# zju3dv/BoxDreamer

Hardware: AMD Instinct MI355X
Metric: poses/s/GPU (5-ref, 224×224, bf16); heatmap max-abs err vs CPU ref (higher is better)
Workload: dtype f16 + e4m3 corrections (BETR q, k columns: f16)

## Files before the change

### boxdreamer_amd/_lib.py

```python
from __future__ import annotations

import ctypes as C
import os
import threading
from typing import NamedTuple

import torch

HERE = os.path.dirname(os.path.abspath(__file__))
LIB_PATH = os.environ.get("BOXDREAMER_HIP_LIB") or os.path.join(HERE, "libboxdreamer_hip.so")

DTYPE_BF16, DTYPE_F16, DTYPE_F32 = 0, 1, 2
PREC_BF16, PREC_F16, PREC_BF16X3, PREC_F16_OUT_BF16X3, PREC_FP8, PREC_BF16_OUT_FP8 = 0, 1, 2, 3, 4, 5
PREC_BF16X3_ATTN_X3 = 6
PREC_F16C8 = 8
PREC_F16_OUT_F16C8, PREC_BF16X3_OUT_F16C8 = 9, 10
PREC_F16C8_QK16 = 13
PREC_F16X3, PREC_F16X3_ATTN_X3 = 14, 15
PREC_F16_OUT_F16X3, PREC_BF16X3_OUT_F16X3 = 16, 17
F16C8_D = 11
PREC_NAMES = {"bf16": PREC_BF16, "fp16": PREC_F16, "f16": PREC_F16, "bf16x3": PREC_BF16X3, "fp8": PREC_FP8,
              "bf16x3_attn_x3": PREC_BF16X3_ATTN_X3, "f16c8": PREC_F16C8, "f16c8_qk16": PREC_F16C8_QK16,
              "f16x3": PREC_F16X3, "f16x3_attn_x3": PREC_F16X3_ATTN_X3}
PREC_NAMES["fp8_mixed"] = PREC_FP8
# ... 60 lines not shown


class BetrWeights(C.Structure):
    _fields_ = [("depth", C.c_int), ("dim", C.c_int), ("heads", C.c_int), ("grid", C.c_int),
                ("patch", C.c_int), ("box_dim", C.c_int), ("kpad", C.c_int),
                ("ln_eps", C.c_float), ("adapter_ln_eps", C.c_float), ("rms_eps", C.c_float),
                ("adapter_fc1", Linear), ("adapter_fc2", Linear), ("bbox_emb", Linear), ("bbox_proj", Linear),
                ("pos_table", C.c_void_p), ("query_token", C.c_void_p),
                ("blocks", C.POINTER(BlockWeights)), ("promote_misc", C.c_int), ("latency_mode", C.c_int)]


class TraceRecord(C.Structure):
    _fields_ = [("kind", C.c_int), ("M", C.c_int), ("N", C.c_int), ("K", C.c_int), ("ms", C.c_float)]


EXPORTS = [
    "bd_abi_version", "bd_target_arch", "bd_gemm", "bd_layernorm", "bd_qk_rmsnorm", "bd_attention",
    "bd_im2col_images", "bd_patchify_heatmaps", "bd_write_prefix_tokens", "bd_query_substitute",
    "bd_gather_query_tokens", "bd_unpatchify_sigmoid", "bd_decode_topk",
    "bd_encoder_workspace_bytes", "bd_encoder_forward", "bd_decoder_workspace_bytes", "bd_decoder_forward",
    "bd_trace_begin", "bd_trace_end", "bd_render_corner_heatmaps", "bd_attention_q", "bd_gather_query_rows_f32",
    "bd_dino_match_scores", "bd_topk_mask", "bd_solve_pnp", "bd_gemm_fuses_qk_rmsnorm", "bd_gemm_takes_ln_fold", "bd_gemm_splitk_flag_bytes",
    "bd_gemm_splitk_workspace_bytes", "bd_solve_pnp_host", "bd_attention_prefix",
    "bd_lanes_prepare", "bd_encoder_workspace_bytes_lanes", "bd_encoder_forward_lanes", "bd_decoder_workspace_bytes_lanes",
    "bd_decoder_forward_lanes", "bd_pose_metrics_workspace_bytes", "bd_pose_metrics", "bd_crop_resize_frames",
    "bd_attention_varlen", "bd_query_substitute_varlen", "bd_gather_query_rows_f32_varlen", "bd_gather_query_tokens_varlen",
    "bd_decoder_workspace_bytes_ragged", "bd_decoder_forward_ragged", "bd_gather_view_rows",
    "bd_match_view_sums", "bd_match_select_rows",
    "bd_assemble_entry_tokens", "bd_decoder_entry_tokens_workspace_bytes", "bd_decoder_entry_tokens",
    "bd_decoder_entry_workspace_bytes", "bd_decoder_forward_entry", "bd_decoder_entry_workspace_bytes_ragged",
    "bd_decoder_forward_entry_ragged", "bd_solve_pnp_wave",
    "bd_solve_pnp_ransac_workspace_bytes", "bd_solve_pnp_ransac_wave", "bd_solve_pnp_ransac_host",
    "bd_round_sources", "bd_pose_select_rows",
]

_lib = None


def load() -> C.CDLL:
    global _lib
    _call.dev = None
    if _lib is not None:
        return _lib
    if not os.path.exists(LIB_PATH):
        raise HipLibraryError(
            f"{LIB_PATH} is missing: the gfx950 HIP kernels are not built. Run "
            "`python -m boxdreamer_amd.build` (or __graft_entry__.build()). There is no CPU/PyTorch fallback.")
    lib = C.CDLL(LIB_PATH)
    for name in EXPORTS:
        if not hasattr(lib, name):
            raise HipLibraryError(f"{LIB_PATH} does not export {name}")
    i, i64, vp, f, sz = C.c_int, C.c_int64, C.c_void_p, C.c_float, C.c_size_t
    lib.bd_abi_version.restype = i
    lib.bd_target_arch.restype = C.c_char_p
    lib.bd_gemm.argtypes = [C.POINTER(GemmArgs), i, vp]
    lib.bd_gemm_fuses_qk_rmsnorm.argtypes = [C.POINTER(GemmArgs), i]
    lib.bd_gemm_takes_ln_fold.argtypes = [C.POINTER(GemmArgs), i]
    lib.bd_gemm_splitk_flag_bytes.argtypes = [i, i]
    lib.bd_gemm_splitk_flag_bytes.restype = sz
    lib.bd_gemm_splitk_workspace_bytes.argtypes = [i, i]
    lib.bd_gemm_splitk_workspace_bytes.restype = sz
    lib.bd_layernorm.argtypes = [vp, i64, vp, vp, f, vp, i64, vp, i64, i, i, i, i, i, i, vp]
    lib.bd_qk_rmsnorm.argtypes = [vp, i64, vp, vp, f, i, i, i, i, vp]
    lib.bd_attention.argtypes = [vp, i64, vp, i64, i, i, i, i, f, i, vp]
    lib.bd_im2col_images.argtypes = [vp, i, vp, i64, i, i, i, i, i, vp]
    lib.bd_patchify_heatmaps.argtypes = [vp, i, vp, i64, i, i, i, i, i, i, vp]
    lib.bd_write_prefix_tokens.argtypes = [vp, vp, i, i, i, i, vp]
    lib.bd_query_substitute.argtypes = [vp, vp, vp, vp, vp, i, i, i, i, vp]
    lib.bd_gather_query_tokens.argtypes = [vp, vp, vp, i64, i, i, i, i, i, vp]
    lib.bd_unpatchify_sigmoid.argtypes = [vp, vp, vp, i, i, i, i, vp]
    lib.bd_decode_topk.argtypes = [vp, i, i, i, i, vp, vp, vp, vp]
    lib.bd_encoder_workspace_bytes.argtypes = [C.POINTER(DinoWeights), i, i]
    lib.bd_encoder_workspace_bytes.restype = sz
    lib.bd_encoder_forward.argtypes = [C.POINTER(DinoWeights), vp, i, i, i, vp, vp, i64, vp, sz, i, vp]
    lib.bd_decoder_workspace_bytes.argtypes = [C.POINTER(BetrWeights), i, i, i]
    lib.bd_decoder_workspace_bytes.restype = sz
    lib.bd_decoder_forward.argtypes = [C.POINTER(BetrWeights), vp, i, vp, i64, vp, i, i, i, vp, vp, vp, sz, i, vp]
    lib.bd_encoder_workspace_bytes_lanes.argtypes = [C.POINTER(DinoWeights), i, i, i]
    lib.bd_encoder_workspace_bytes_lanes.restype = sz
    lib.bd_encoder_forward_lanes.argtypes = [C.POINTER(DinoWeights), vp, i, i, i, vp, vp, i64, vp, sz, i, i, vp]
    lib.bd_decoder_workspace_bytes_lanes.argtypes = [C.POINTER(BetrWeights), i, i, i, i]
    lib.bd_decoder_workspace_bytes_lanes.restype = sz
    lib.bd_decoder_forward_lanes.argtypes = [C.POINTER(BetrWeights), vp, i, vp, i64, vp, i, i, i, vp, vp, vp, sz, i, i, vp]
    lib.bd_lanes_prepare.argtypes = []
    lib.bd_attention_q.argtypes = [vp, i64, vp, i64, i, i, i, i, f, vp, i, i, vp]
    lib.bd_attention_prefix.argtypes = [vp, i64, vp, i64, i, i, i, i, f, i, i, i, vp]
    lib.bd_gather_query_rows_f32.argtypes = [vp, vp, vp, i, i, i, i, vp]
    lib.bd_render_corner_heatmaps.argtypes = [vp, i, i, i, i, vp, i, vp]
    lib.bd_dino_match_scores.argtypes = [vp, vp, i, vp, i, i, i, i, i, i, f, vp, vp, vp, vp]
    lib.bd_topk_mask.argtypes = [vp, i, i, i, vp, vp]
# ... 291 lines not shown
```

### boxdreamer_amd/csrc/bd_common.h

```cpp
#pragma once
#include <hip/hip_runtime.h>
#include <stdint.h>

#include "../../include/boxdreamer_hip.h"

typedef __attribute__((__vector_size__(8 * sizeof(__bf16)))) __bf16 bf16x8;
typedef __attribute__((__vector_size__(8 * sizeof(_Float16)))) _Float16 f16x8;
typedef __attribute__((__vector_size__(16 * sizeof(float)))) float f32x16;
typedef __attribute__((__vector_size__(4 * sizeof(float)))) float f32x4;
typedef __attribute__((__vector_size__(16))) unsigned int u128;

template <class T> struct Op16;
template <> struct Op16<__bf16> {
    typedef bf16x8 vec8;
    static __device__ __forceinline__ f32x16 mfma(vec8 a, vec8 b, f32x16 c) {
        return __builtin_amdgcn_mfma_f32_32x32x16_bf16(a, b, c, 0, 0, 0);
    }
};
template <> struct Op16<_Float16> {
    typedef f16x8 vec8;
    static __device__ __forceinline__ f32x16 mfma(vec8 a, vec8 b, f32x16 c) {
        return __builtin_amdgcn_mfma_f32_32x32x16_f16(a, b, c, 0, 0, 0);
    }
};
// ... 286 lines not shown
            }
            if (beta) {
                const float4 bb = *(const float4*)(beta + c);
                y[0] += bb.x; y[1] += bb.y; y[2] += bb.z; y[3] += bb.w;
            }
            if (out32_row) *(float4*)(out32_row + c) = make_float4(y[0], y[1], y[2], y[3]);
            if (out16) {
                if constexpr (__is_same(T, f16c8)) {
                    f16c8_store4(out16, out16_plane, orow * cols + c, y);
                } else if constexpr (NS == 2) {
                    float hi4[4], lo4[4];
#pragma unroll
                    for (int j = 0; j < 4; ++j) split_hi_lo<T>(y[j], hi4[j], lo4[j]);
                    store_cvt<T, 4>(out16 + orow * cols + c, hi4);
                    store_cvt<T, 4>(out16 + out16_plane + orow * cols + c, lo4);
                } else {
                    store_cvt<T, 4>(out16 + orow * cols + c, y);
                }
            }
        }
    }
}

template <class T, int NS, bool NT>
__device__ __forceinline__ void ln_row(const float* __restrict__ xr, const float* __restrict__ gamma, const float* __restrict__ beta,
                                       float eps, T* __restrict__ out16, int64_t out16_plane, float* __restrict__ out32_row,
                                       int64_t orow, int cols, int lane) {
    f32x4 t[4];
    ln_row_load<NT>(xr, cols, lane, t);
    ln_row_finish<T, NS>(t, gamma, beta, eps, out16, out16_plane, out32_row, orow, cols, lane);
}

int& bd_concurrent_launches();

int bd_attention_q_forms(const void* qkv, int64_t qkv_plane, void* out, int64_t out_plane, int batch, int seq, int heads, int head_dim,
                         float scale, const int32_t* q_view, int q_len, int prec, int latency_forms, void* stream);

int bd_assemble_entry_tokens_from(const float* bank_x, int bank_views, const float* rgb_fresh, int fresh_first, int n_fresh, const float* pos,
                                  const float* query_token, const int32_t* src, float* x_out, int n_views, int P, int dim, void* stream);

int bd_trace_open(hipStream_t s, int kind, int M, int N, int K);
void bd_trace_close(hipStream_t s, int slot);

#define BD_CHECK_LAUNCH() do { hipError_t e__ = hipGetLastError(); if (e__ != hipSuccess) return (int)e__; } while (0)
```

### boxdreamer_amd/csrc/gemm_common.h

```cpp
#pragma once
#include "bd_common.h"
#include <type_traits>

#ifdef BD_GEMM_PROBE
static __device__ unsigned* bd_probe_buf = nullptr;
#define BD_PROBE(idx) { const unsigned long long t__ = __builtin_amdgcn_s_memtime(); if ((idx) < 64) probe_ts = (lane == (idx)) ? (unsigned)t__ : probe_ts; }
#define BD_PROBE_IF(c, idx) { if (c) BD_PROBE(idx) }
#define BD_PROBE_RT(idx) { const unsigned long long t__ = __builtin_amdgcn_s_memrealtime(); probe_ts = (lane == (idx)) ? (unsigned)t__ : probe_ts; }
#else
#define BD_PROBE(idx)
#define BD_PROBE_IF(c, idx)
#define BD_PROBE_RT(idx)
#endif


namespace {


template <int CH> __device__ __forceinline__ int swz_chunk(int row, int c) {
    constexpr int RPB = 16 / CH;
    return c ^ ((row / RPB) & (CH - 1));
}

template <int BM_, int BN_>
// ... 654 lines not shown
    const float m[8] = {st[0][0], st[0][2], st[1][0], st[1][2], st[2][0], st[2][2], st[3][0], st[3][2]};
    const float q[8] = {st[0][1], st[0][3], st[1][1], st[1][3], st[2][1], st[2][3], st[3][1], st[3][3]};
    float mean = 0.f, m2 = 0.f;
#pragma unroll
    for (int i = 0; i < 8; ++i) mean += m[i];
    mean *= 0.125f;
#pragma unroll
    for (int i = 0; i < 8; ++i) { const float d = m[i] - mean; m2 += q[i] + 96.0f * (d * d); }
    const float rstd = rsqrtf(m2 * (1.0f / 768.0f) + eps);
    return make_float2(rstd, -mean * rstd);
}
inline bool ln_fold_producer(const bd_gemm_args& a) { return a.ln_stats_out != nullptr || a.ln_op_out != nullptr || a.ln_resid_in_op != 0; }
inline bool ln_fold_consumer(const bd_gemm_args& a) { return a.ln_stats_in != nullptr || a.ln_colsum != nullptr; }
inline bool ln_fold_producer_ok(const bd_gemm_args& a) {
    if (a.ln_resid_in_op ? (a.resid != nullptr || (a.out_f32 != OUT_F32 && a.out_f32 != OUT_OPERAND)) : a.out_f32 != OUT_F32) return false;
    return a.ln_stats_out && a.ln_op_out && a.N == 768 && a.act == BD_ACT_NONE && !a.rms_wq && !a.addtab && a.rpg_in <= 0 &&
           !a.wscale && a.ln_op_ld % 32 == 0 && a.ln_op_plane % 8 == 0 && (((uintptr_t)a.ln_op_out | (uintptr_t)a.ln_stats_out) & 15) == 0 &&
           (int64_t)a.M * a.ln_op_ld < ((int64_t)1 << 30);
}
inline bool ln_fold_consumer_ok(const bd_gemm_args& a) {
    return a.ln_stats_in && a.ln_colsum && a.K == 768 && a.N % 192 == 0 && a.out_f32 != OUT_F32 && !a.resid && !a.addtab && a.rpg_in <= 0 && !a.wscale &&
           a.bias && (((uintptr_t)a.ln_stats_in | (uintptr_t)a.ln_colsum | (uintptr_t)a.bias) & 15) == 0;
}

inline bool wide_epilogue_ok(const bd_gemm_args& p, int ns) {
    return (p.N % 8 == 0) && (p.ldo % 8 == 0) && (((uintptr_t)p.out & 15) == 0) &&
           (!p.resid || ((p.ldr % 4 == 0) && ((uintptr_t)p.resid & 15) == 0)) &&
           (!p.bias || ((uintptr_t)p.bias & 15) == 0) && (!p.addtab || ((uintptr_t)p.addtab & 15) == 0) &&
           (!p.wscale || ((uintptr_t)p.wscale & 15) == 0) && (p.out_f32 || ns == 1 || (p.out_plane % 8 == 0));
}


inline int cu_count() {
    static int cached[16] = {0};
    int dev = 0;
    if (hipGetDevice(&dev) != hipSuccess || dev < 0 || dev >= 16) return 256;
    if (cached[dev] == 0) {
        int n = 0;
        if (hipDeviceGetAttribute(&n, hipDeviceAttributeMultiprocessorCount, dev) != hipSuccess || n <= 0) n = 256;
        cached[dev] = n;
    }
    return cached[dev];
}

inline bool rms_geometry_ok(const bd_gemm_args& a) {
    return a.rms_wq && a.rms_wk && a.out_f32 != OUT_F32 && a.act == BD_ACT_NONE && !a.resid && !a.addtab && a.rpg_in <= 0 &&
           (a.rms_parts == 0 || a.rms_parts == 2 || a.rms_parts == 3) &&
           a.N % (a.rms_parts == 2 ? 2 : 3) == 0 && (a.N / (a.rms_parts == 2 ? 2 : 3)) % 96 == 0 && a.N % 192 == 0 && (((uintptr_t)a.rms_wq | (uintptr_t)a.rms_wk) & 3) == 0;
}

}

inline int64_t pc192_main_rows(const bd_gemm_args& a, int cus) {
    if (a.rms_wq || a.addtab || a.rpg_in > 0) return a.M;
    const int64_t tn = a.N / 192, mt = (a.M + 255) / 256, nt = mt * tn;
    const int64_t k = nt / cus, rem = nt % cus;
    if (k < 1 || k > 4 || rem == 0 || rem * 4 > cus) return a.M;
    const int64_t rows = (k * cus / tn) * 256;
    return rows > 0 ? rows : a.M;
}

int bd_launch_gemm_f16c8(const bd_gemm_args& a, hipStream_t s);
bool bd_f16c8_takes_ln_fold(const bd_gemm_args& a);
```

### boxdreamer_amd/csrc/gemm_f16c8.hip

```cpp
#include "gemm_common.h"

#ifdef BD_GEMM_PROBE
extern "C" int bd_gemm_f16c8_probe_set(void* buf) {
    return (int)hipMemcpyToSymbol(HIP_SYMBOL(bd_probe_buf), &buf, sizeof(buf));
}
#endif

namespace {

template <int NSTAGE, int EP, int OUTK, bool GELU, int WM = 4, int WN = 2, int NPW = 4, bool LNF = false, bool SK = false>
__global__ __launch_bounds__((WM * WN + NPW) * 64, (WM * WN + NPW) <= 4 ? 2 : 1) void gemm_kernel_pc_f16c8(const bd_gemm_args p) {
    constexpr int MI = 2, NI = 3, NCW = WM * WN;
    constexpr int TBM = WM * MI * 32, TBN = WN * NI * 32, BK = 32;
    constexpr int A0 = TBM * 64, W0 = TBN * 64, A1 = TBM * 32, W1 = TBN * 64;
    constexpr int OFF_W0 = A0, OFF_A1 = A0 + W0, OFF_W1 = A0 + W0 + A1, STAGE = A0 + W0 + A1 + W1;
    constexpr int SR = 16, SCRATCH = NCW * SR * NI * 32 * 4, S2 = SCRATCH > STAGE ? SCRATCH : STAGE;
    static_assert(SCRATCH <= STAGE, "the epilogue scratch overlays stage 2");
    constexpr int GA0 = TBM / 16, GW0 = TBN / 16, GA1 = TBM / 32, GW1 = TBN / 16;
    constexpr int IA0 = (GA0 + NPW - 1) / NPW, IW0 = (GW0 + NPW - 1) / NPW, IA1 = (GA1 + NPW - 1) / NPW, IW1 = (GW1 + NPW - 1) / NPW;
    static_assert(GA0 % NPW == 0 && GW0 % NPW == 0 && GA1 % NPW == 0 && GW1 % NPW == 0, "every producer wave issues the same number of pieces (counted vmcnt)");
    constexpr int PIECES = IA0 + IW0 + IA1 + IW1;
    constexpr int WAIT_ONE_SLAB = (PIECES & 15) | ((PIECES >> 4) << 14) | 0x70 | 0xF00;
    constexpr int AUX_COLP = 2 * STAGE + S2, AUX_RMS = AUX_COLP + 4096, AUX_ROWS = AUX_RMS + 2048, AUX_BYTES = EP == 0 ? 0 : (LNF ? 10240 : 6144);
    static_assert(!LNF || (EP != 0 && NPW * 64 >= TBM && NSTAGE == 3), "LayerNorm fold: one producer lane per tile row");
// ... 344 lines not shown
                          (ep == 2 && outk == OUT_F16);
        if (!form) return false;
    }
    return true;
}

static int f16c8_split_k(const bd_gemm_args& a, int ep, bool r5, bool lnp, bool s3, int cus) {
    (void)lnp;
    if (!a.sk_ws || ((uintptr_t)a.sk_ws & 255) || !s3 || a.N % 96 != 0 || !bd_gemm_splitk_flag_bytes(a.M, a.N) || !(ep == 3 || r5)) return 1;
    const int t96 = ((a.M + 127) / 128) * (a.N / 96), nk = a.K / 32;
    const int slots = cus / (bd_concurrent_launches() > 0 ? bd_concurrent_launches() : 1);
    int sk = a.sk_split;
    if (sk <= 0) {
        sk = 1;
        for (int c = 4; c >= 2; --c)
            if (t96 * c <= slots && nk / c >= 6) { sk = c; break; }
    }
    if (sk < 2 || sk > 4 || nk / sk < 1) return 1;
    return sk;
}

extern "C" size_t bd_gemm_splitk_flag_bytes(int M, int N) {
    if (M <= 0 || N <= 0 || N % 96 != 0 || M > BD_SPLITK_MAX_ROWS) return 0;
    const size_t t96 = (size_t)((M + 127) / 128) * (size_t)(N / 96);
    return t96 * 3 * 2 * 4 <= BD_SPLITK_FLAG_BYTES ? BD_SPLITK_FLAG_BYTES : 0;
}
extern "C" size_t bd_gemm_splitk_workspace_bytes(int M, int N) {
    const size_t fb = bd_gemm_splitk_flag_bytes(M, N);
    if (!fb) return 0;
    const size_t t96 = (size_t)((M + 127) / 128) * (size_t)(N / 96);
    return fb + t96 * 3 * 2 * (size_t)(64 * 96 * 4);
}

int bd_launch_gemm_f16c8(const bd_gemm_args& a, hipStream_t s) {
    if (!wide_epilogue_ok(a, 2) || 256 * a.lda * 2 >= ((int64_t)1 << 31) || 256 * a.ldw * 2 >= ((int64_t)1 << 31)) return BD_ERR_ALIGN;
    if ((a.K % 32) || (a.lda % 32) || (a.ldw % 32)) return BD_ERR_SHAPE;
    if (a.out_f32 == OUT_OPERAND && (a.ldo % 32)) return BD_ERR_SHAPE;
    if (a.w_qexp + BD_F16C8_D < -100 || a.w_qexp + BD_F16C8_D > 120) return BD_ERR_SHAPE;
    if (a.rms_wq && !rms_geometry_ok(a)) return BD_ERR_SHAPE;
    const bool lnp = ln_fold_producer(a), lnc = ln_fold_consumer(a);
    if ((lnp || lnc) && !bd_f16c8_takes_ln_fold(a)) return BD_ERR_SHAPE;
    const int slot = bd_trace_open(s, 0, a.M, a.N, a.K);
    const int cus = cu_count();
    const int tiles = ((a.M + 255) / 256) * ((a.N + 191) / 192);
    int outk = 0;
    bool gelu = false;
    const int ep = f16c8_epilogue_kind(a, outk, gelu);
    const bool s3 = (a.K / 32) % 3 == 0;
    const int tiles_small = ((a.M + 127) / 128) * ((a.N + 191) / 192);
    const bool small = s3 && ep != 0 && 2 * tiles * bd_concurrent_launches() <= cus;
    const bool small0 = ep == 0 && 2 * tiles * bd_concurrent_launches() <= cus;
    const dim3 g0(tiles_small < cus ? tiles_small : cus);
    const int grid = small ? (tiles_small < cus ? tiles_small : cus) : (tiles < cus ? tiles : cus);
    const dim3 g(grid), b(small ? 512 : 768);
#define BD_C8_LAUNCH(EP_, OUTK_, GELU_)                                                                     \
    { if (small) hipLaunchKernelGGL((gemm_kernel_pc_f16c8<3, EP_, OUTK_, GELU_, 2, 2, 4>), g, b, 0, s, a);     \
      else if (s3) hipLaunchKernelGGL((gemm_kernel_pc_f16c8<3, EP_, OUTK_, GELU_>), g, b, 0, s, a);            \
      else hipLaunchKernelGGL((gemm_kernel_pc_f16c8<2, EP_, OUTK_, GELU_>), g, b, 0, s, a); }
#define BD_C8_LAUNCH_LN(EP_, OUTK_, GELU_, LNF_)                                                                        \
    { if (small) hipLaunchKernelGGL((gemm_kernel_pc_f16c8<3, EP_, OUTK_, GELU_, 2, 2, 4, LNF_>), g, b, 0, s, a);         \
      else hipLaunchKernelGGL((gemm_kernel_pc_f16c8<3, EP_, OUTK_, GELU_, 4, 2, 4, LNF_>), g, b, 0, s, a); }
    const bool r5 = lnp && a.ln_resid_in_op;
    const bool fc2_96 = (ep == 3 || r5) && small && a.K >= 2048 && a.N % 96 == 0 && 4 * tiles * bd_concurrent_launches() <= cus;
    const int sk = f16c8_split_k(a, ep, r5, lnp, s3, cus);
    if (sk > 1) {
        bd_gemm_args b2 = a;
        b2.sk_split = sk;
        const int t96 = ((a.M + 127) / 128) * (a.N / 96);
        const dim3 gs(((t96 + 7) / 8) * 8 * sk), bs(256);
        if (r5 && a.out_f32 == OUT_F32) hipLaunchKernelGGL((gemm_kernel_pc_f16c8<3, 5, OUT_F32, false, 2, 1, 2, false, true>), gs, bs, 0, s, b2);
        else if (r5) hipLaunchKernelGGL((gemm_kernel_pc_f16c8<3, 5, OUT_OPERAND, false, 2, 1, 2, false, true>), gs, bs, 0, s, b2);
        else if (lnp) hipLaunchKernelGGL((gemm_kernel_pc_f16c8<3, 4, OUT_F32, false, 2, 1, 2, false, true>), gs, bs, 0, s, b2);
        else hipLaunchKernelGGL((gemm_kernel_pc_f16c8<3, 3, OUT_F32, false, 2, 1, 2, false, true>), gs, bs, 0, s, b2);
        bd_trace_close(s, slot);
        BD_CHECK_LAUNCH();
        return BD_OK;
    }
    if (r5 && fc2_96 && a.out_f32 == OUT_F32)
        hipLaunchKernelGGL((gemm_kernel_pc_f16c8<3, 5, OUT_F32, false, 2, 1, 2>), dim3(((a.M + 127) / 128) * (a.N / 96)), dim3(256), 0, s, a);
    else if (r5 && fc2_96)
        hipLaunchKernelGGL((gemm_kernel_pc_f16c8<3, 5, OUT_OPERAND, false, 2, 1, 2>), dim3(((a.M + 127) / 128) * (a.N / 96)), dim3(256), 0, s, a);
    else if (r5 && a.out_f32 == OUT_F32) BD_C8_LAUNCH_LN(5, OUT_F32, false, false)
    else if (r5) BD_C8_LAUNCH_LN(5, OUT_OPERAND, false, false)
    else if (lnp && fc2_96)
        hipLaunchKernelGGL((gemm_kernel_pc_f16c8<3, 4, OUT_F32, false, 2, 1, 2>), dim3(((a.M + 127) / 128) * (a.N / 96)), dim3(256), 0, s, a);
    else if (lnp) BD_C8_LAUNCH_LN(4, OUT_F32, false, false)
    else if (lnc && ep == 1 && gelu) BD_C8_LAUNCH_LN(1, OUT_OPERAND, true, true)
    else if (lnc && ep == 1 && outk == OUT_F16) BD_C8_LAUNCH_LN(1, OUT_F16, false, true)
    else if (lnc && ep == 1) BD_C8_LAUNCH_LN(1, OUT_BF16X2, false, true)
    else if (lnc) BD_C8_LAUNCH_LN(2, OUT_F16, false, true)
    else if (fc2_96)
        hipLaunchKernelGGL((gemm_kernel_pc_f16c8<3, 3, OUT_F32, false, 2, 1, 2>), dim3(((a.M + 127) / 128) * (a.N / 96)), dim3(256), 0, s, a);
    else if (ep == 3) BD_C8_LAUNCH(3, OUT_F32, false)
    else if (ep == 2 && outk == OUT_OPERAND) BD_C8_LAUNCH(2, OUT_OPERAND, false)
    else if (ep == 2 && outk == OUT_F16) BD_C8_LAUNCH(2, OUT_F16, false)
    else if (ep == 2) BD_C8_LAUNCH(2, OUT_BF16X2, false)
    else if (ep == 1 && gelu) BD_C8_LAUNCH(1, OUT_OPERAND, true)
    else if (ep == 1 && outk == OUT_OPERAND) BD_C8_LAUNCH(1, OUT_OPERAND, false)
    else if (ep == 1 && outk == OUT_F16) BD_C8_LAUNCH(1, OUT_F16, false)
    else if (ep == 1) BD_C8_LAUNCH(1, OUT_BF16X2, false)
    else if (small0 && s3) hipLaunchKernelGGL((gemm_kernel_pc_f16c8<3, 0, OUT_OPERAND, false, 2, 2, 4>), g0, dim3(512), 0, s, a);
    else if (small0) hipLaunchKernelGGL((gemm_kernel_pc_f16c8<2, 0, OUT_OPERAND, false, 2, 2, 4>), g0, dim3(512), 0, s, a);
    else if (s3) hipLaunchKernelGGL((gemm_kernel_pc_f16c8<3, 0, OUT_OPERAND, false>), g, b, 0, s, a);
    else hipLaunchKernelGGL((gemm_kernel_pc_f16c8<2, 0, OUT_OPERAND, false>), g, b, 0, s, a);
#undef BD_C8_LAUNCH
#undef BD_C8_LAUNCH_LN
    bd_trace_close(s, slot);
    BD_CHECK_LAUNCH();
    return BD_OK;
}
```

### include/boxdreamer_hip.h

```cpp
#ifndef BOXDREAMER_HIP_H
#define BOXDREAMER_HIP_H

#include <stddef.h>
#include <stdint.h>

#ifdef __cplusplus
extern "C" {
#endif

#define BD_ABI_VERSION 9

#define BD_DTYPE_BF16 0
#define BD_DTYPE_F16 1
#define BD_DTYPE_F32 2

#define BD_PREC_BF16 0
#define BD_PREC_F16 1
#define BD_PREC_BF16X3 2
#define BD_PREC_F16_OUT_BF16X3 3
#define BD_PREC_FP8 4
#define BD_PREC_BF16_OUT_FP8 5
#define BD_PREC_BF16X3_ATTN_X3 6
#define BD_PREC_F16C8 8
#define BD_PREC_F16C8_QK16 13
// ... 14 lines not shown
#define BD_ACT_NONE 0
#define BD_ACT_GELU 1

int bd_abi_version(void);
const char* bd_target_arch(void);


typedef struct bd_gemm_args {
    const void* A; int64_t lda; int64_t a_plane;
    const void* W; int64_t ldw; int64_t w_plane;
    const float* bias;
    const float* wscale;
    const float* resid; int64_t ldr;
    const float* addtab; int tab_rows;
    void* out; int64_t ldo; int64_t out_plane;
    int out_f32;
    int M, N, K;
    int act;
    int rpg_in, rpg_out, row_off;
    int w_qexp;
    const float* rms_wq; const float* rms_wk; float rms_eps;
    int rms_parts;
    float* ln_stats_out; void* ln_op_out; int64_t ln_op_plane; int64_t ln_op_ld;
    const float* ln_stats_in; const float* ln_colsum; float ln_eps;
    int ln_resid_in_op;
    void* sk_ws; int sk_split;
} bd_gemm_args;
#define BD_SPLITK_MAX_ROWS 4096
#define BD_SPLITK_FLAG_BYTES 16384
size_t bd_gemm_splitk_flag_bytes(int M, int N);
size_t bd_gemm_splitk_workspace_bytes(int M, int N);
int bd_gemm(const bd_gemm_args* args , int prec, void* stream);
int bd_gemm_takes_ln_fold(const bd_gemm_args* args , int prec);
int bd_gemm_fuses_qk_rmsnorm(const bd_gemm_args* args , int prec);

int bd_layernorm(const float* x, int64_t ldx, const float* gamma, const float* beta, float eps,
                 void* out16, int64_t out16_plane, float* out32, int64_t ldo, int rows, int cols,
                 int rpg_in, int rpg_out, int row_off, int prec, void* stream);

int bd_qk_rmsnorm(void* qkv, int64_t plane, const float* wq, const float* wk, float eps, int rows,
                  int heads, int head_dim, int prec, void* stream);

int bd_attention(const void* qkv, int64_t qkv_plane, void* out, int64_t out_plane, int batch, int seq,
                 int heads, int head_dim, float scale, int prec, void* stream);

int bd_attention_q(const void* qkv, int64_t qkv_plane, void* out, int64_t out_plane, int batch, int seq,
                   int heads, int head_dim, float scale, const int32_t* q_view, int q_len, int prec, void* stream);

int bd_attention_prefix(const void* qkv, int64_t qkv_plane, void* out, int64_t out_plane, int batch, int seq, int heads,
                        int head_dim, float scale, int n_prefix, int prefix_queries, int prec, void* stream);

int bd_attention_varlen(const void* qkv, int64_t qkv_plane, void* out, int64_t out_plane, const int32_t* view_start, int batch,
                        int n_views, int max_views, int tokens_per_view, int heads, int head_dim, float scale,
                        const int32_t* q_view, int prec, void* stream);

int bd_im2col_images(const void* images, int img_dtype, void* out16, int64_t out_plane, int n_images,
                     int size, int patch, int kpad, int prec, void* stream);

int bd_patchify_heatmaps(const void* heat, int in_dtype, void* out16, int64_t out_plane, int n_images,
                         int channels, int size, int patch, int kpad, int prec, void* stream);

int bd_write_prefix_tokens(float* x, const float* prefix, int n_images, int tokens_per_image,
                           int n_prefix, int dim, void* stream);

int bd_query_substitute(float* x, const float* rgb, const float* pos, const float* query_token,
                        const int32_t* query_idx, int B, int T, int P, int dim, void* stream);
// ... 180 lines not shown
```

### boxdreamer_amd/csrc/attention.hip

```cpp
#include "bd_common.h"
#include <type_traits>

#ifdef BD_ATTN_PROBE
__device__ unsigned* bd_attn_probe_buf = nullptr;
extern "C" int bd_attn_probe_set(void* buf) { return (int)hipMemcpyToSymbol(HIP_SYMBOL(bd_attn_probe_buf), &buf, sizeof(buf)); }
#define AP(idx) { const unsigned long long t__ = __builtin_amdgcn_s_memtime(); if ((idx) < 64) probe_ts = (lane == (idx)) ? (unsigned)t__ : probe_ts; }
#else
#define AP(idx) {}
#endif

namespace {

struct AttnArgs {
    const void* qkv; int64_t qkv_plane;
    void* out; int64_t out_plane;
    int batch, seq, heads;
    float scale_log2e;
    const int32_t* q_view;
    int q_len;
    int q_off;
    int out_rows;
    const int32_t* view_start;
    int tpv, n_views, max_views;
};
// ... 4 lines not shown
        const int i = i0 + lane;
        const bool below = i < batch && (int64_t)view_start[i + 1] * ipv <= (int64_t)wg;
        b += __popcll(__ballot(below));
    }
    return __builtin_amdgcn_readfirstlane(b);
}

constexpr int KT = 64;

__device__ __forceinline__ int vswz(int d) { return ((d >> 1) ^ (d >> 4)) & 7; }

__device__ __forceinline__ unsigned pack_lo16(unsigned a, unsigned b) { return __builtin_amdgcn_perm(b, a, 0x05040100u); }
__device__ __forceinline__ unsigned pack_hi16(unsigned a, unsigned b) { return __builtin_amdgcn_perm(b, a, 0x07060302u); }

template <class T, int NS, int HD, int NW, int OUTMODE = 0, bool VL = false>
__global__ __launch_bounds__(NW * 64, NS == 1 && HD == 64 ? 3 : 2) void attn_kernel(const AttnArgs p) {
    bd_saturating_conversions();
    typedef typename Op16<T>::vec8 vec8;
    constexpr int NT = NW * 64;
    constexpr int DCH = HD / 8;
    constexpr int KSTRIDE = HD * 2 + 16;
    constexpr int K_BYTES = KT * KSTRIDE;
    constexpr int V_BYTES = HD * 128;
    constexpr int PLANE_BYTES = K_BYTES + V_BYTES;
    constexpr int KCH = KT * DCH;
    constexpr int KCPT = (KCH + NT - 1) / NT;
    constexpr int VMT = (KT / 4) * DCH;
    static_assert(VMT <= NT, "one V micro-tile per thread");
    constexpr int QB = NW * 32;
    constexpr int DM = HD / 32;
    constexpr int KS = HD / 16;
    constexpr int BUF_BYTES = NS * PLANE_BYTES;
    constexpr int NBUF = NS == 1 ? 2 : 1;
    __shared__ __attribute__((aligned(16))) unsigned char lds[NBUF * BUF_BYTES];

    const int tid = threadIdx.x, lane = tid & 63, wid = tid >> 6;
#ifdef BD_ATTN_PROBE
    unsigned probe_ts = 0;
    AP(60)
#endif
    const int lq = lane & 31, lh = lane >> 5;
    int seq = p.seq;
    const int heads = p.heads;
    int q_len = p.q_len;
    int nqb = (q_len + QB - 1) / QB;

    int wg;
    {
        const int nwg = gridDim.x, bid = blockIdx.x, xcd = bid & 7, q = nwg >> 3, r = nwg & 7;
        wg = (xcd < r ? xcd * (q + 1) : r * (q + 1) + (xcd - r) * q) + (bid >> 3);
    }
    int qb = wg % nqb;
    int bh = wg / nqb;
    int head = bh % heads, b = bh / heads;
    int64_t row0 = (int64_t)b * seq;
    int vl_views = 0;
    if constexpr (VL) {
        if (!p.q_view) {
            const int ipv = (p.tpv / QB) * heads;
            b = vl_sample_of(p.view_start, p.batch, ipv, wg, lane);
            if (b >= p.batch) return;
        }
        const int s0 = __builtin_amdgcn_readfirstlane(p.view_start[b]), s1 = __builtin_amdgcn_readfirstlane(p.view_start[b + 1]);
        vl_views = s1 - s0;
        if (s0 < 0 || vl_views <= 0 || vl_views > p.max_views || s1 > p.n_views) return;
        seq = vl_views * p.tpv;
        row0 = (int64_t)s0 * p.tpv;
// ... 2 lines not shown
            nqb = vl_views * (p.tpv / QB);
            const int local = wg - s0 * (p.tpv / QB) * heads;
            qb = local % nqb;
            head = local / nqb;
        }
    }

    const int ld = 3 * heads * HD;
    const T* base = (const T*)p.qkv + row0 * ld + head * HD;
    const T* qbase = base;
    const T* kbase = base + heads * HD;
    const T* vbase = base + 2 * heads * HD;
    const int64_t plane = p.qkv_plane;

    const int q0 = qb * QB + wid * 32;
    int qbase_row = p.q_view ? p.q_view[b] * q_len : p.q_off;
    if constexpr (VL) { if (p.q_view) { const int qv = p.q_view[b]; qbase_row = (qv < 0 ? 0 : (qv < vl_views ? qv : vl_views - 1)) * q_len; } }
    int qrow = q0 + lq; qrow = (qrow < q_len ? qrow : q_len - 1) + qbase_row;
    auto out_row0 = [&]() -> int64_t {
        if constexpr (VL) { if (!p.q_view) return row0; }
        return (int64_t)b * p.out_rows + (p.out_rows == q_len ? 0 : p.q_off);
    };
    vec8 qf[NS][KS];
#pragma unroll
    for (int s = 0; s < NS; ++s)
#pragma unroll
        for (int ks = 0; ks < KS; ++ks)
            qf[s][ks] = as_vec8<T>(*(const u128*)(qbase + s * plane + (unsigned)(qrow * ld + ks * 16 + lh * 8)));

    int kc_row[KCPT], kc_col[KCPT];
    unsigned kc_off[KCPT];
#pragma unroll
    for (int i = 0; i < KCPT; ++i) {
        const int c = tid + NT * i;
        kc_row[i] = c / DCH;
        kc_col[i] = c % DCH;
        kc_off[i] = (unsigned)(kc_row[i] * ld + kc_col[i] * 8);
    }
    const int vm_kq = tid / DCH, vm_dc = tid % DCH;
    const bool vm_active = tid < VMT;
    const unsigned vm_off = (unsigned)(vm_kq * 4 * ld + vm_dc * 8);
    const bool ragged = (seq % KT) != 0;
    int vdst;
    {
        const int g = vm_kq >> 2, qi = vm_kq & 3;
        const int qp = (qi == 1) ? 2 : (qi == 2 ? 1 : qi);
        vdst = ((g * 2 + (qp >> 1)) << 4) | ((qp & 1) << 3);
    }

    u128 rk[NS][KCPT], rv[NS][4];
    __amdgpu_buffer_rsrc_t rsrc[NS];
    {
        const int bytes = __builtin_amdgcn_readfirstlane(seq * ld * (int)sizeof(T));
#pragma unroll
        for (int s = 0; s < NS; ++s) {
            const uintptr_t a = (uintptr_t)(base + s * plane);
            const unsigned lo = __builtin_amdgcn_readfirstlane((unsigned)a), hi = __builtin_amdgcn_readfirstlane((unsigned)(a >> 32));
            rsrc[s] = __builtin_amdgcn_make_buffer_rsrc((void*)(((uintptr_t)hi << 32) | lo), 0, bytes, 0x00020000);
        }
    }
    const int row_bytes = __builtin_amdgcn_readfirstlane(ld * (int)sizeof(T));
    int k_voff[KCPT];
#pragma unroll
    for (int i = 0; i < KCPT; ++i) k_voff[i] = ((int)kc_off[i] + heads * HD) * (int)sizeof(T);
    const int v_voff = ((int)vm_off + 2 * heads * HD) * (int)sizeof(T);
#define LOAD_TILE(kt)                                                                         \
    _Pragma("unroll") for (int s = 0; s < NS; ++s) {                                          \
        _Pragma("unroll") for (int i = 0; i < KCPT; ++i) {                                    \
            if (KCH % NT == 0 || tid + NT * i < KCH)                                          \
                rk[s][i] = __builtin_bit_cast(u128, __builtin_amdgcn_raw_buffer_load_b128(rsrc[s], k_voff[i], (kt) * KT * row_bytes, 0)); \
        }                                                                                     \
        if (vm_active) {                                                                      \
            _Pragma("unroll") for (int j = 0; j < 4; ++j)                                     \
                rv[s][j] = __builtin_bit_cast(u128, __builtin_amdgcn_raw_buffer_load_b128(rsrc[s], v_voff, ((kt) * KT + j) * row_bytes, 0)); \
        }                                                                                     \
    }
#define STORE_TILE(buf)                                                                        \
    _Pragma("unroll") for (int s = 0; s < NS; ++s) {                                          \
        unsigned char* kl = lds + (buf) * BUF_BYTES + s * PLANE_BYTES;                        \
        unsigned char* vl = kl + K_BYTES;                                                     \
        _Pragma("unroll") for (int i = 0; i < KCPT; ++i)                                      \
            if (KCH % NT == 0 || tid + NT * i < KCH)                                          \
                *(u128*)(kl + kc_row[i] * KSTRIDE + kc_col[i] * 16) = rk[s][i];               \
        if (vm_active) {                                                                      \
            _Pragma("unroll") for (int w = 0; w < 4; ++w) {                                   \
                const unsigned a0 = rv[s][0][w], a1 = rv[s][1][w], a2 = rv[s][2][w], a3 = rv[s][3][w]; \
                const int d = vm_dc * 8 + 2 * w;                                              \
                uint2 lo, hi;                                                                 \
                lo.x = pack_lo16(a0, a1); lo.y = pack_lo16(a2, a3);       \
                hi.x = pack_hi16(a0, a1); hi.y = pack_hi16(a2, a3); \
                *(uint2*)(vl + d * 128 + (vdst ^ (vswz(d) << 4))) = lo;                \
                *(uint2*)(vl + (d + 1) * 128 + (vdst ^ (vswz(d + 1) << 4))) = hi;    \
            }                                                                                 \
        }                                                                                     \
    }

    f32x16 oacc[DM];
#pragma unroll
    for (int i = 0; i < DM; ++i)
#pragma unroll
        for (int r = 0; r < 16; ++r) oacc[i][r] = 0.f;
    float m_run = -INFINITY, l_run = 0.f;
    const float sc = p.scale_log2e;

    const int nt = (seq + KT - 1) / KT;
    LOAD_TILE(0)
    STORE_TILE(0)
    __syncthreads();
    AP(61)
    const bool small_tail = HD == 64 && nt > 1 && seq % KT != 0 && seq % KT <= 16;
    auto tile = [&](const int kt, auto tail_c) {
        constexpr int TAIL = decltype(tail_c)::value;
        constexpr int KMN = TAIL == 2 ? 1 : 2, GN = TAIL == 2 ? 1 : 4;
        if (kt + 1 < nt) { LOAD_TILE(kt + 1) }
        const unsigned char* cur = lds + (NBUF == 2 ? (kt & 1) : 0) * BUF_BYTES;
        if (kt < 7) AP(kt * 8)

        f32x16 sacc[KMN];
#pragma unroll
        for (int km = 0; km < KMN; ++km) {
#pragma unroll
            for (int r = 0; r < 16; ++r) sacc[km][r] = 0.f;
#pragma unroll
            for (int ks = 0; ks < KS; ++ks) {
                vec8 kf[NS];
#pragma unroll
                for (int s = 0; s < NS; ++s)
                    kf[s] = as_vec8<T>(*(const u128*)(cur + s * PLANE_BYTES + (km * 32 + lq) * KSTRIDE + (ks * 2 + lh) * 16));
                if (NS == 2) {
                    sacc[km] = Op16<T>::mfma(kf[NS - 1], qf[0][ks], sacc[km]);
                    sacc[km] = Op16<T>::mfma(kf[0], qf[NS - 1][ks], sacc[km]);
                }
                sacc[km] = Op16<T>::mfma(kf[0], qf[0][ks], sacc[km]);
            }
        }
        if (kt < 7) AP(kt * 8 + 1)
        float tmax = -INFINITY;
        if (TAIL == 2 || (kt + 1) * KT > seq) {
#pragma unroll
            for (int km = 0; km < KMN; ++km)
#pragma unroll
                for (int r = 0; r < 16; ++r) {
                    const int key = kt * KT + km * 32 + (r & 3) + 8 * (r >> 2) + 4 * lh;
                    if (key >= seq) sacc[km][r] = -INFINITY;
                }
        }
#pragma unroll
        for (int km = 0; km < KMN; ++km)
#pragma unroll
            for (int r = 0; r < 16; ++r) tmax = fmaxf(tmax, sacc[km][r]);
        tmax = fmaxf(tmax, __shfl_xor(tmax, 32));
        const float m_new = fmaxf(m_run, tmax);
        if (!__all(m_new == m_run)) {
            const float alpha = __builtin_amdgcn_exp2f((m_run - m_new) * sc);
            l_run *= alpha;
#pragma unroll
            for (int i = 0; i < DM; ++i)
#pragma unroll
                for (int r = 0; r < 16; ++r) oacc[i][r] *= alpha;
            m_run = m_new;
        }
        const float mneg = -m_run * sc;
        float psum = 0.f;
#pragma unroll
        for (int km = 0; km < KMN; ++km)
#pragma unroll
            for (int r = 0; r < 16; ++r) {
                const float pv = __builtin_amdgcn_exp2f(fmaf(sacc[km][r], sc, mneg));
                sacc[km][r] = pv;
                psum += pv;
            }
        l_run += psum;
        if (kt < 7) AP(kt * 8 + 2)

#pragma unroll
        for (int g = 0; g < GN; ++g) {
            vec8 pf[NS];
#pragma unroll
            for (int j = 0; j < 8; ++j) {
                const float pv = sacc[g >> 1][(g & 1) * 8 + j];
                const T hi = from_f32<T>(pv);
                pf[0][j] = hi;
                if (NS == 2) pf[NS - 1][j] = from_f32<T>(pv - to_f32<T>(hi));
            }
#pragma unroll
            for (int dm = 0; dm < DM; ++dm) {
                const int d = dm * 32 + lq;
                vec8 vf[NS];
#pragma unroll
                for (int s = 0; s < NS; ++s)
                    vf[s] = as_vec8<T>(*(const u128*)(cur + s * PLANE_BYTES + K_BYTES + d * 128 +
                                                        (((g * 2 + lh) ^ vswz(d)) << 4)));
                if (NS == 2) {
                    oacc[dm] = Op16<T>::mfma(vf[NS - 1], pf[0], oacc[dm]);
                    oacc[dm] = Op16<T>::mfma(vf[0], pf[NS - 1], oacc[dm]);
                }
                oacc[dm] = Op16<T>::mfma(vf[0], pf[0], oacc[dm]);
            }
        }
        if (kt < 7) AP(kt * 8 + 3)
        if (NBUF == 1) __syncthreads();
        if (kt < 7) AP(kt * 8 + 4)
        if (kt + 1 < nt) { STORE_TILE(NBUF == 2 ? ((kt + 1) & 1) : 0) }
        if (kt < 7) AP(kt * 8 + 5)
        __syncthreads();
        if (kt < 7) AP(kt * 8 + 6)
    };
    for (int kt = 0; kt < nt - (small_tail ? 1 : 0); ++kt) tile(kt, std::integral_constant<int, 0>{});
    if (small_tail) tile(nt - 1, std::integral_constant<int, 2>{});
#undef LOAD_TILE
#undef STORE_TILE

    AP(62)
    const float l_tot = l_run + __shfl_xor(l_run, 32);
    const float inv = 1.0f / l_tot;
    const int q = q0 + lq;
    if (q < q_len) {
        if (OUTMODE == 2) {
            fp8e4* orow = (fp8e4*)p.out + (out_row0() + q) * (heads * HD) + head * HD;
#pragma unroll
            for (int dm = 0; dm < DM; ++dm)
#pragma unroll
                for (int rq = 0; rq < 4; ++rq) {
                    float v4[4];
#pragma unroll
                    for (int j = 0; j < 4; ++j) v4[j] = oacc[dm][rq * 4 + j] * inv;
                    store_cvt<fp8e4, 4>(orow + dm * 32 + 8 * rq + 4 * lh, v4);
                }
        } else if (OUTMODE == 3) {
            const int64_t e0 = (out_row0() + q) * (heads * HD) + head * HD;
#pragma unroll
            for (int dm = 0; dm < DM; ++dm)
#pragma unroll
                for (int rq = 0; rq < 4; ++rq) {
                    float v4[4];
#pragma unroll
                    for (int j = 0; j < 4; ++j) v4[j] = oacc[dm][rq * 4 + j] * inv;
                    f16c8_store4((f16c8*)p.out, p.out_plane, e0 + dm * 32 + 8 * rq + 4 * lh, v4);
                }
        } else if (OUTMODE == 1 || OUTMODE == 4) {
            typedef typename std::conditional<OUTMODE == 1, __bf16, _Float16>::type OT;
            OT* orow = (OT*)p.out + (out_row0() + q) * (heads * HD) + head * HD;
// ... 517 lines not shown
```

Measured before the change: 736.4.

## Split f16c8 GEMM into main and tail row launches to fix wave quantization

When the f16c8 GEMM tile count leaves a small partial final wave across CUs, the GEMM is split by rows into two launches. The main launch covers a whole number of waves and the tail launch can pick a different, smaller-tile form. This targets the idle-CU cost of a mostly empty last wave on output-f32 and LN-producer epilogues. It adds a second launch per affected GEMM. A CU-count and concurrency override plus a query export are added for testing.

```diff
diff --git a/boxdreamer_amd/_lib.py b/boxdreamer_amd/_lib.py
--- a/boxdreamer_amd/_lib.py
+++ b/boxdreamer_amd/_lib.py
@@ -116,6 +116,7 @@
     "bd_decoder_forward_entry_ragged", "bd_solve_pnp_wave",
     "bd_solve_pnp_ransac_workspace_bytes", "bd_solve_pnp_ransac_wave", "bd_solve_pnp_ransac_host",
     "bd_round_sources", "bd_pose_select_rows",
+    "bd_gemm_launch_model_override", "bd_gemm_f16c8_main_rows",
 ]
 
 _lib = None
@@ -140,6 +141,9 @@
     lib.bd_gemm.argtypes = [C.POINTER(GemmArgs), i, vp]
     lib.bd_gemm_fuses_qk_rmsnorm.argtypes = [C.POINTER(GemmArgs), i]
     lib.bd_gemm_takes_ln_fold.argtypes = [C.POINTER(GemmArgs), i]
+    lib.bd_gemm_launch_model_override.argtypes = [i, i]
+    lib.bd_gemm_f16c8_main_rows.argtypes = [C.POINTER(GemmArgs)]
+    lib.bd_gemm_f16c8_main_rows.restype = i64
     lib.bd_gemm_splitk_flag_bytes.argtypes = [i, i]
     lib.bd_gemm_splitk_flag_bytes.restype = sz
     lib.bd_gemm_splitk_workspace_bytes.argtypes = [i, i]
diff --git a/boxdreamer_amd/csrc/bd_common.h b/boxdreamer_amd/csrc/bd_common.h
--- a/boxdreamer_amd/csrc/bd_common.h
+++ b/boxdreamer_amd/csrc/bd_common.h
@@ -342,6 +342,7 @@
 }
 
 int& bd_concurrent_launches();
+int& bd_cu_count_override();
 
 int bd_attention_q_forms(const void* qkv, int64_t qkv_plane, void* out, int64_t out_plane, int batch, int seq, int heads, int head_dim,
                          float scale, const int32_t* q_view, int q_len, int prec, int latency_forms, void* stream);
diff --git a/boxdreamer_amd/csrc/gemm_common.h b/boxdreamer_amd/csrc/gemm_common.h
--- a/boxdreamer_amd/csrc/gemm_common.h
+++ b/boxdreamer_amd/csrc/gemm_common.h
@@ -710,6 +710,7 @@
 
 
 inline int cu_count() {
+    if (bd_cu_count_override() > 0) return bd_cu_count_override();
     static int cached[16] = {0};
     int dev = 0;
     if (hipGetDevice(&dev) != hipSuccess || dev < 0 || dev >= 16) return 256;
@@ -738,5 +739,14 @@
     return rows > 0 ? rows : a.M;
 }
 
+inline int64_t f16c8_main_rows(const bd_gemm_args& a, int cus) {
+    if (a.rms_wq || a.addtab || a.rpg_in > 0 || a.ln_stats_in || a.ln_colsum || a.N % 192 || cus <= 0) return a.M;
+    const int64_t tn = a.N / 192, mt = (a.M + 255) / 256, nt = mt * tn;
+    const int64_t k = nt / cus, rem = nt % cus;
+    if (k < 1 || k > 4 || rem == 0 || rem * 4 > cus) return a.M;
+    const int64_t rows = (k * cus / tn) * 256;
+    return rows > 0 && rows < a.M ? rows : a.M;
+}
+
 int bd_launch_gemm_f16c8(const bd_gemm_args& a, hipStream_t s);
 bool bd_f16c8_takes_ln_fold(const bd_gemm_args& a);
diff --git a/boxdreamer_amd/csrc/gemm_f16c8.hip b/boxdreamer_amd/csrc/gemm_f16c8.hip
--- a/boxdreamer_amd/csrc/gemm_f16c8.hip
+++ b/boxdreamer_amd/csrc/gemm_f16c8.hip
@@ -400,16 +400,85 @@
     return fb + t96 * 3 * 2 * (size_t)(64 * 96 * 4);
 }
 
-int bd_launch_gemm_f16c8(const bd_gemm_args& a, hipStream_t s) {
+int& bd_cu_count_override() {
+    static thread_local int n = 0;
+    return n;
+}
+
+static int f16c8_check_args(const bd_gemm_args& a) {
     if (!wide_epilogue_ok(a, 2) || 256 * a.lda * 2 >= ((int64_t)1 << 31) || 256 * a.ldw * 2 >= ((int64_t)1 << 31)) return BD_ERR_ALIGN;
     if ((a.K % 32) || (a.lda % 32) || (a.ldw % 32)) return BD_ERR_SHAPE;
     if (a.out_f32 == OUT_OPERAND && (a.ldo % 32)) return BD_ERR_SHAPE;
     if (a.w_qexp + BD_F16C8_D < -100 || a.w_qexp + BD_F16C8_D > 120) return BD_ERR_SHAPE;
     if (a.rms_wq && !rms_geometry_ok(a)) return BD_ERR_SHAPE;
-    const bool lnp = ln_fold_producer(a), lnc = ln_fold_consumer(a);
-    if ((lnp || lnc) && !bd_f16c8_takes_ln_fold(a)) return BD_ERR_SHAPE;
+    if ((ln_fold_producer(a) || ln_fold_consumer(a)) && !bd_f16c8_takes_ln_fold(a)) return BD_ERR_SHAPE;
+    return BD_OK;
+}
+
+static bd_gemm_args f16c8_row_slice(const bd_gemm_args& a, int64_t row0, int rows) {
+    bd_gemm_args sub = a;
+    sub.M = rows;
+    sub.sk_ws = nullptr;
+    sub.sk_split = 0;
+    sub.A = (const unsigned char*)a.A + row0 * a.lda * 2;
+    sub.a_plane = a.a_plane - row0 * a.lda / 2;
+    if (a.out) {
+        sub.out = (unsigned char*)a.out + row0 * a.ldo * (a.out_f32 == OUT_F32 ? 4 : 2);
+        if (a.out_f32 == OUT_OPERAND) sub.out_plane = a.out_plane - row0 * a.ldo / 2;
+    }
+    if (a.resid) sub.resid = a.resid + row0 * a.ldr;
+    if (a.ln_op_out) {
+        sub.ln_op_out = (unsigned char*)a.ln_op_out + row0 * a.ln_op_ld * 2;
+        sub.ln_op_plane = a.ln_op_plane - row0 * a.ln_op_ld / 2;
+    }
+    if (a.ln_stats_out) sub.ln_stats_out = a.ln_stats_out + row0 * (a.N / 96) * 2;
+    return sub;
+}
+
+static int64_t f16c8_tail_split_rows(const bd_gemm_args& a, int cus) {
+    int outk = 0;
+    bool gelu = false;
+    const int ep = f16c8_epilogue_kind(a, outk, gelu);
+    const bool s3 = (a.K / 32) % 3 == 0, lnp = ln_fold_producer(a), r5 = lnp && a.ln_resid_in_op;
+    if (!s3 || !(ep == 3 || lnp) || ln_fold_consumer(a) || bd_concurrent_launches() > 1) return a.M;
+    if (f16c8_split_k(a, ep, r5, lnp, s3, cus) > 1) return a.M;
+    const int64_t rows = f16c8_main_rows(a, cus);
+    if (rows >= a.M) return a.M;
+    if (lnp && !(ln_fold_producer_ok(f16c8_row_slice(a, 0, (int)rows)) && ln_fold_producer_ok(f16c8_row_slice(a, rows, (int)(a.M - rows))))) return a.M;
+    return rows;
+}
+
+static void f16c8_launch_form(const bd_gemm_args& a, hipStream_t s, int cus);
+
+int bd_launch_gemm_f16c8(const bd_gemm_args& a, hipStream_t s) {
+    const int rc = f16c8_check_args(a);
+    if (rc != BD_OK) return rc;
     const int slot = bd_trace_open(s, 0, a.M, a.N, a.K);
     const int cus = cu_count();
+    const int64_t rows_main = f16c8_tail_split_rows(a, cus);
+    if (rows_main < a.M) {
+        f16c8_launch_form(f16c8_row_slice(a, 0, (int)rows_main), s, cus);
+        f16c8_launch_form(f16c8_row_slice(a, rows_main, (int)(a.M - rows_main)), s, cus);
+    } else
+        f16c8_launch_form(a, s, cus);
+    bd_trace_close(s, slot);
+    BD_CHECK_LAUNCH();
+    return BD_OK;
+}
+
+extern "C" int bd_gemm_launch_model_override(int cus, int lanes) {
+    bd_cu_count_override() = cus > 0 ? cus : 0;
+    bd_concurrent_launches() = lanes > 1 ? lanes : 1;
+    return BD_OK;
+}
+extern "C" int64_t bd_gemm_f16c8_main_rows(const bd_gemm_args* args) {
+    if (!args) return 0;
+    if (f16c8_check_args(*args) != BD_OK) return args->M;
+    return f16c8_tail_split_rows(*args, cu_count());
+}
+
+static void f16c8_launch_form(const bd_gemm_args& a, hipStream_t s, int cus) {
+    const bool lnp = ln_fold_producer(a), lnc = ln_fold_consumer(a);
     const int tiles = ((a.M + 255) / 256) * ((a.N + 191) / 192);
     int outk = 0;
     bool gelu = false;
@@ -440,9 +509,7 @@
         else if (r5) hipLaunchKernelGGL((gemm_kernel_pc_f16c8<3, 5, OUT_OPERAND, false, 2, 1, 2, false, true>), gs, bs, 0, s, b2);
         else if (lnp) hipLaunchKernelGGL((gemm_kernel_pc_f16c8<3, 4, OUT_F32, false, 2, 1, 2, false, true>), gs, bs, 0, s, b2);
         else hipLaunchKernelGGL((gemm_kernel_pc_f16c8<3, 3, OUT_F32, false, 2, 1, 2, false, true>), gs, bs, 0, s, b2);
-        bd_trace_close(s, slot);
-        BD_CHECK_LAUNCH();
-        return BD_OK;
+        return;
     }
     if (r5 && fc2_96 && a.out_f32 == OUT_F32)
         hipLaunchKernelGGL((gemm_kernel_pc_f16c8<3, 5, OUT_F32, false, 2, 1, 2>), dim3(((a.M + 127) / 128) * (a.N / 96)), dim3(256), 0, s, a);
@@ -473,7 +540,4 @@
     else hipLaunchKernelGGL((gemm_kernel_pc_f16c8<2, 0, OUT_OPERAND, false>), g, b, 0, s, a);
 #undef BD_C8_LAUNCH
 #undef BD_C8_LAUNCH_LN
-    bd_trace_close(s, slot);
-    BD_CHECK_LAUNCH();
-    return BD_OK;
-}
+}
diff --git a/include/boxdreamer_hip.h b/include/boxdreamer_hip.h
--- a/include/boxdreamer_hip.h
+++ b/include/boxdreamer_hip.h
@@ -70,6 +70,8 @@
 size_t bd_gemm_splitk_workspace_bytes(int M, int N);
 int bd_gemm(const bd_gemm_args* args , int prec, void* stream);
 int bd_gemm_takes_ln_fold(const bd_gemm_args* args , int prec);
+int bd_gemm_launch_model_override(int cus, int lanes);
+int64_t bd_gemm_f16c8_main_rows(const bd_gemm_args* args );
 int bd_gemm_fuses_qk_rmsnorm(const bd_gemm_args* args , int prec);
 
 int bd_layernorm(const float* x, int64_t ldx, const float* gamma, const float* beta, float eps,
```

Measured after the change: 738.9 (median of 2 runs). Within noise of the previous version (+0.3%).

## Stage small attention tail tile into dedicated LDS up front and drop its barrier

Applied to the files above, without the earlier changes.

When the key sequence ends in a small ragged tail (at most 16 keys, HD 64), wave 2 now loads that tail's K and V at kernel start into a separate LDS region. The last two tiles then run without the load, store and __syncthreads steps of the pipeline. The tail tile also reads a compact 16-row K layout and a 32-byte V stride. K-load indexing is changed so that out-of-range threads reload a duplicate chunk instead of branching. Together these remove one staged iteration's barrier and LDS round trip plus per-thread predicates, at the cost of extra LDS for the tail buffer, which may reduce occupancy.

```diff
diff --git a/boxdreamer_amd/csrc/attention.hip b/boxdreamer_amd/csrc/attention.hip
--- a/boxdreamer_amd/csrc/attention.hip
+++ b/boxdreamer_amd/csrc/attention.hip
@@ -60,7 +60,10 @@
     constexpr int KS = HD / 16;
     constexpr int BUF_BYTES = NS * PLANE_BYTES;
     constexpr int NBUF = NS == 1 ? 2 : 1;
-    __shared__ __attribute__((aligned(16))) unsigned char lds[NBUF * BUF_BYTES];
+    constexpr int TK_BYTES = 16 * KSTRIDE, TV_BYTES = HD * 32, TPLANE_BYTES = TK_BYTES + TV_BYTES;
+    constexpr int TAIL_BYTES = HD == 64 ? NS * TPLANE_BYTES : 0;
+    static_assert(HD != 64 || (NW >= 3 && VMT <= 128), "the tail is staged by wave 2, which holds no V micro-tile");
+    __shared__ __attribute__((aligned(16))) unsigned char lds[NBUF * BUF_BYTES + TAIL_BYTES];
 
     const int tid = threadIdx.x, lane = tid & 63, wid = tid >> 6;
 #ifdef BD_ATTN_PROBE
@@ -129,7 +132,7 @@
     unsigned kc_off[KCPT];
 #pragma unroll
     for (int i = 0; i < KCPT; ++i) {
-        const int c = tid + NT * i;
+        const int c = tid + NT * i - ((KCH % NT != 0 && tid + NT * i >= KCH) ? NT : 0);
         kc_row[i] = c / DCH;
         kc_col[i] = c % DCH;
         kc_off[i] = (unsigned)(kc_row[i] * ld + kc_col[i] * 8);
@@ -163,10 +166,8 @@
     const int v_voff = ((int)vm_off + 2 * heads * HD) * (int)sizeof(T);
 #define LOAD_TILE(kt)                                                                         \
     _Pragma("unroll") for (int s = 0; s < NS; ++s) {                                          \
-        _Pragma("unroll") for (int i = 0; i < KCPT; ++i) {                                    \
-            if (KCH % NT == 0 || tid + NT * i < KCH)                                          \
-                rk[s][i] = __builtin_bit_cast(u128, __builtin_amdgcn_raw_buffer_load_b128(rsrc[s], k_voff[i], (kt) * KT * row_bytes, 0)); \
-        }                                                                                     \
+        _Pragma("unroll") for (int i = 0; i < KCPT; ++i)                                      \
+            rk[s][i] = __builtin_bit_cast(u128, __builtin_amdgcn_raw_buffer_load_b128(rsrc[s], k_voff[i], (kt) * KT * row_bytes, 0)); \
         if (vm_active) {                                                                      \
             _Pragma("unroll") for (int j = 0; j < 4; ++j)                                     \
                 rv[s][j] = __builtin_bit_cast(u128, __builtin_amdgcn_raw_buffer_load_b128(rsrc[s], v_voff, ((kt) * KT + j) * row_bytes, 0)); \
@@ -177,8 +178,7 @@
         unsigned char* kl = lds + (buf) * BUF_BYTES + s * PLANE_BYTES;                        \
         unsigned char* vl = kl + K_BYTES;                                                     \
         _Pragma("unroll") for (int i = 0; i < KCPT; ++i)                                      \
-            if (KCH % NT == 0 || tid + NT * i < KCH)                                          \
-                *(u128*)(kl + kc_row[i] * KSTRIDE + kc_col[i] * 16) = rk[s][i];               \
+            *(u128*)(kl + kc_row[i] * KSTRIDE + kc_col[i] * 16) = rk[s][i];                   \
         if (vm_active) {                                                                      \
             _Pragma("unroll") for (int w = 0; w < 4; ++w) {                                   \
                 const unsigned a0 = rv[s][0][w], a1 = rv[s][1][w], a2 = rv[s][2][w], a3 = rv[s][3][w]; \
@@ -201,16 +201,58 @@
     const float sc = p.scale_log2e;
 
     const int nt = (seq + KT - 1) / KT;
+    const bool small_tail = HD == 64 && nt > 1 && seq % KT != 0 && seq % KT <= 16;
+    const bool tail_wave = small_tail && __builtin_amdgcn_readfirstlane(wid) == 2;
+    const int t4 = (lane & 31) >> 3, c8 = lane & 7;
     LOAD_TILE(0)
+    if constexpr (HD == 64) {
+        if (tail_wave) {
+            const int t_voff = (t4 * 4 * ld + c8 * 8 + (lh ? 1 : 2) * heads * HD) * (int)sizeof(T);
+#pragma unroll
+            for (int s = 0; s < NS; ++s)
+#pragma unroll
+                for (int j = 0; j < 4; ++j)
+                    rv[s][j] = __builtin_bit_cast(u128, __builtin_amdgcn_raw_buffer_load_b128(rsrc[s], t_voff, ((nt - 1) * KT + j) * row_bytes, 0));
+        }
+    }
     STORE_TILE(0)
+    if constexpr (HD == 64) {
+        if (tail_wave) {
+            const int qp = (t4 == 1) ? 2 : (t4 == 2 ? 1 : t4);
+            const int tvdst = ((qp >> 1) << 4) | ((qp & 1) << 3);
+#pragma unroll
+            for (int s = 0; s < NS; ++s) {
+                unsigned char* tk = lds + NBUF * BUF_BYTES + s * TPLANE_BYTES;
+                unsigned char* tv = tk + TK_BYTES;
+                if (lh) {
+#pragma unroll
+                    for (int j = 0; j < 4; ++j) *(u128*)(tk + (t4 * 4 + j) * KSTRIDE + c8 * 16) = rv[s][j];
+                } else {
+#pragma unroll
+                    for (int w = 0; w < 4; ++w) {
+                        const unsigned a0 = rv[s][0][w], a1 = rv[s][1][w], a2 = rv[s][2][w], a3 = rv[s][3][w];
+                        const int d = c8 * 8 + 2 * w;
+                        uint2 lo, hi;
+                        lo.x = pack_lo16(a0, a1); lo.y = pack_lo16(a2, a3);
+                        hi.x = pack_hi16(a0, a1); hi.y = pack_hi16(a2, a3);
+                        *(uint2*)(tv + d * 32 + tvdst) = lo;
+                        *(uint2*)(tv + (d + 1) * 32 + tvdst) = hi;
+                    }
+                }
+            }
+        }
+    }
     __syncthreads();
     AP(61)
-    const bool small_tail = HD == 64 && nt > 1 && seq % KT != 0 && seq % KT <= 16;
-    auto tile = [&](const int kt, auto tail_c) {
+    auto tile = [&](const int kt, auto tail_c, auto stage_c) {
         constexpr int TAIL = decltype(tail_c)::value;
+        constexpr bool STAGE = decltype(stage_c)::value;
+        static_assert(TAIL == 0 || !STAGE, "the peeled tail is never staged");
         constexpr int KMN = TAIL == 2 ? 1 : 2, GN = TAIL == 2 ? 1 : 4;
-        if (kt + 1 < nt) { LOAD_TILE(kt + 1) }
-        const unsigned char* cur = lds + (NBUF == 2 ? (kt & 1) : 0) * BUF_BYTES;
+        constexpr int PSTRIDE = TAIL == 2 ? TPLANE_BYTES : PLANE_BYTES;
+        constexpr int VOFF = TAIL == 2 ? TK_BYTES : K_BYTES;
+        if (STAGE && kt + 1 < nt) { LOAD_TILE(kt + 1) }
+        const unsigned char* cur = TAIL == 2 ? lds + NBUF * BUF_BYTES : lds + (NBUF == 2 ? (kt & 1) : 0) * BUF_BYTES;
         if (kt < 7) AP(kt * 8)
 
         f32x16 sacc[KMN];
@@ -223,7 +265,7 @@
                 vec8 kf[NS];
 #pragma unroll
                 for (int s = 0; s < NS; ++s)
-                    kf[s] = as_vec8<T>(*(const u128*)(cur + s * PLANE_BYTES + (km * 32 + lq) * KSTRIDE + (ks * 2 + lh) * 16));
+                    kf[s] = as_vec8<T>(*(const u128*)(cur + s * PSTRIDE + (TAIL == 2 ? (lq & 15) : km * 32 + lq) * KSTRIDE + (ks * 2 + lh) * 16));
                 if (NS == 2) {
                     sacc[km] = Op16<T>::mfma(kf[NS - 1], qf[0][ks], sacc[km]);
                     sacc[km] = Op16<T>::mfma(kf[0], qf[NS - 1][ks], sacc[km]);
@@ -233,7 +275,7 @@
         }
         if (kt < 7) AP(kt * 8 + 1)
         float tmax = -INFINITY;
-        if (TAIL == 2 || (kt + 1) * KT > seq) {
+        if (TAIL == 2 || (STAGE && (kt + 1) * KT > seq)) {
 #pragma unroll
             for (int km = 0; km < KMN; ++km)
 #pragma unroll
@@ -286,8 +328,8 @@
                 vec8 vf[NS];
 #pragma unroll
                 for (int s = 0; s < NS; ++s)
-                    vf[s] = as_vec8<T>(*(const u128*)(cur + s * PLANE_BYTES + K_BYTES + d * 128 +
-                                                        (((g * 2 + lh) ^ vswz(d)) << 4)));
+                    vf[s] = as_vec8<T>(*(const u128*)(cur + s * PSTRIDE + VOFF + (TAIL == 2 ? d * 32 + (lh << 4)
+                                                                                             : d * 128 + (((g * 2 + lh) ^ vswz(d)) << 4))));
                 if (NS == 2) {
                     oacc[dm] = Op16<T>::mfma(vf[NS - 1], pf[0], oacc[dm]);
                     oacc[dm] = Op16<T>::mfma(vf[0], pf[NS - 1], oacc[dm]);
@@ -296,15 +338,22 @@
             }
         }
         if (kt < 7) AP(kt * 8 + 3)
-        if (NBUF == 1) __syncthreads();
+        if (STAGE && NBUF == 1) __syncthreads();
         if (kt < 7) AP(kt * 8 + 4)
-        if (kt + 1 < nt) { STORE_TILE(NBUF == 2 ? ((kt + 1) & 1) : 0) }
+        if (STAGE && kt + 1 < nt) { STORE_TILE(NBUF == 2 ? ((kt + 1) & 1) : 0) }
         if (kt < 7) AP(kt * 8 + 5)
-        __syncthreads();
+        if (STAGE) __syncthreads();
         if (kt < 7) AP(kt * 8 + 6)
     };
-    for (int kt = 0; kt < nt - (small_tail ? 1 : 0); ++kt) tile(kt, std::integral_constant<int, 0>{});
-    if (small_tail) tile(nt - 1, std::integral_constant<int, 2>{});
+    const std::integral_constant<int, 0> any_tile{};
+    const int n_staged = small_tail ? nt - 2 : nt;
+    for (int kt = 0; kt < n_staged; ++kt) tile(kt, any_tile, std::true_type{});
+    if constexpr (HD == 64) {
+        if (small_tail) {
+            tile(nt - 2, any_tile, std::false_type{});
+            tile(nt - 1, std::integral_constant<int, 2>{}, std::false_type{});
+        }
+    }
 #undef LOAD_TILE
 #undef STORE_TILE
 
```

New measurement: 776.8 before, 780.7 after (median of 6 runs). About the same (+0.5%).
